# juicedata/juicefs

Measured on AMD Instinct MI355X. Metric: device-resident GiB/s (de)compress, 4 MiB blocks, LZ4+Zstd, 1/2/4/8 MI355X, higher is better.
Workload: dtype u8; 1 GPU; LZ4 decompress, 4096x4MiB blocks already in HBM (BASELINE configs[1]); blocks_per_gpu=4096, block_bytes=4194304, class=T, compressed_bytes_per_gpu=8570049795, parallelism=1 process(es), one per GPU, blocks sharded, no collective

## Files before the change

### juicefs_amd/csrc/lz4_decode.hip

```cpp
#include <hip/hip_runtime.h>
#include <stdint.h>

#include "jfs_internal.h"
#include "lz4_put16.h"
#include "lz4_tailpack.h"
#include "lz4_walkstep.h"
#include "wave.cuh"

namespace jfs {
namespace lz4d {

constexpr int P = 32;
constexpr int CW = 64 * P;
constexpr int CWIN = CW + 80;
constexpr int R = 4096;
constexpr int RMASK = R - 1;
constexpr int SEG = 128;
constexpr int TMAX = CW / 3 + 2;
constexpr int TCAP = 448 < TMAX ? 448 : TMAX;
#ifndef JFS_DIAG
#define JFS_DIAG 0
#endif
enum : unsigned {
    D_SKIP_ZERO = 1,
    D_SKIP_LIT = 2,
    D_SKIP_FAR = 4,
    D_SKIP_SUBST = 8,
    D_SKIP_NEAR = 16,
    D_PARSEONLY = 32,
    D_NOCOPY = 64,
};
constexpr unsigned DIAG = JFS_DIAG;
constexpr uint32_t STOP = 0x80000000u;
constexpr uint32_t NONE = 0xFFFFFFFFu;
constexpr int KEXT = 64;
constexpr int FLUSH_T = 1024;
constexpr int LMAX = 64;
constexpr int BSPAN = 2048;
static_assert(BSPAN + FLUSH_T + 128 <= R, "ring must hold the unflushed tail plus one batch");
static_assert(R - BSPAN >= LMAX + 16, "far sources must lie below the flushed prefix");
static_assert(R == (int)TP_RING && LMAX <= (int)TP_LEN_MAX, "tail_pack field widths (lz4_tailpack.h)");

#ifdef JFS_PROF
#define NPROF 30
__device__ uint64_t g_prof[NPROF];
struct Prof {
    uint64_t t, last, acc[NPROF];
    __device__ void start() {
        t = __builtin_amdgcn_s_memtime();
        for (int i = 0; i < NPROF; i++) acc[i] = 0;
    }
    __device__ void stamp(int k) {
        uint64_t x = __builtin_amdgcn_s_memtime();
        last = x - t;
        acc[k] += last;
        t = x;
    }
    __device__ void flush_out() {
        if (__lane_id() == 0)
            for (int i = 0; i < NPROF; i++) atomicAdd((unsigned long long *)&g_prof[i], acc[i]);
    }
};
#define PSTAMP(k) pr.stamp(k)
#define PCOUNT(k, n) (pr.acc[k] += (n))
#define PFIRST(...) __VA_ARGS__
#define PWALK(kind)                                                        \
    do {                                                                   \
        const uint64_t re_ = __ballot((kind) == WS_REDONE);                \
        pr.acc[26] += (uint64_t)__popcll(re_);                             \
        pr.acc[27] += re_ != 0;                                            \
        pr.acc[28] += (uint64_t)__popcll(__ballot((kind) == WS_ARRIVED)); \
    } while (0)
#define PROF_ARG , Prof &pr
#define PROF_PASS , pr
#else
#define PSTAMP(k)
#define PCOUNT(k, n)
#define PFIRST(...)
#define PWALK(kind) (void)(kind)
#define PROF_ARG
#define PROF_PASS
#endif

enum { W_NONE = 0, W_WIN = 1, W_SER = 2, W_BUG = 3 };
constexpr int32_t W_PFIRST = 16;
struct Meta {
    int32_t kind, wbase, cbase;
    uint32_t T, efin;
};
struct Ctl {
    int32_t done, restart, rip;
    int32_t step;
};

struct Smem {
    alignas(16) uint8_t ring[R];
    alignas(16) uint8_t cwin[2][CWIN];
    alignas(16) uint16_t tab[2][TCAP];
    Meta meta[2];
    Ctl ctl;
};

struct Ctx {
    const gc_u8 *src;
    g_u8 *dst;
    int32_t n;
    int32_t cap;
    int32_t F;
    int32_t Fw;
    uint32_t dmis;
    int32_t cbase;
    int32_t bug;
    uint8_t *cw;
    uint32_t cwoff;
    uint16_t *tab;
};

typedef uint32_t u32x4 __attribute__((ext_vector_type(4), aligned(4)));
typedef uint32_t u32x2 __attribute__((ext_vector_type(2), aligned(4)));
typedef JFS_GLOBAL const u32x4 gc_x4;
typedef JFS_GLOBAL const u32x2 gc_x2;

__device__ __forceinline__ uint32_t slot(const Ctx &c, int32_t pos) { return (uint32_t)(pos + (int32_t)c.dmis) & RMASK; }

template <bool UNDER>
__device__ __forceinline__ void far_load(const Ctx &c, uintptr_t a, uint32_t &d0, uint32_t &d1, uint32_t &d2,
                                         uint32_t &d3, uint32_t &d4, uint32_t &d5) {
    const uintptr_t b = a & ~(uintptr_t)3, lo = (uintptr_t)c.dst & ~(uintptr_t)3;
    const bool under = UNDER && b < lo;
    const gc_x4 *q = (const gc_x4 *)(under ? lo : b);
    const u32x4 v = q[0];
    const u32x2 w = *(const gc_x2 *)(q + 1);
    d0 = v.x; d1 = v.y; d2 = v.z; d3 = v.w; d4 = w.x; d5 = w.y;
    if (under) { d5 = d4; d4 = d3; d3 = d2; d2 = d1; d1 = d0; d0 = 0; }
}

__device__ __forceinline__ uint32_t cb(const Smem &s, const Ctx &c, int32_t p) {
    int32_t r = p - c.cbase;
    if ((uint32_t)r < (uint32_t)CWIN) return c.cw[r];
    return (p >= 0 && p < c.n) ? c.src[p] : 0u;
}

__device__ __forceinline__ void stage_window(Smem &s, Ctx &c, int32_t wbase) {
    const int l = lane_id();
    const uint32_t mis = (uint32_t)(((uintptr_t)c.src + (uint32_t)wbase) & 15u);
    c.cbase = wbase - (int32_t)mis;
    constexpr int NCH = (CWIN / 16 + 63) / 64;
    uint4 v[NCH];
#pragma unroll
    for (int j = 0; j < NCH; ++j) {
        const int k = l + 64 * j;
        const int32_t p = c.cbase + 16 * k;
        v[j] = make_uint4(0, 0, 0, 0);
        if (k < CWIN / 16 && p < c.n) v[j] = *(const gc_u4 *)(c.src + p);
    }
#pragma unroll
    for (int j = 0; j < NCH; ++j) {
        const int k = l + 64 * j;
        if (k < CWIN / 16) *(uint4 *)(c.cw + 16 * k) = v[j];
    }
    if (c.cbase < 0 || c.cbase + CWIN > c.n) {
        for (int k = l; k < CWIN; k += 64) {
            int32_t p = c.cbase + k;
            if (p >= c.n || p < 0) c.cw[k] = 0;
        }
    }
}

struct Tok {
    int32_t nxt;
    int32_t ll;
    int32_t ml;
    int32_t off;
    int32_t lit;
    int32_t llx;
};

__device__ __forceinline__ Tok parse_tok(const Smem &s, const Ctx &c, int32_t p) {
    Tok t;
    const int32_t n = c.n;
    t.ll = t.ml = t.off = t.lit = t.llx = 0;
    if (p > n - 18) { t.nxt = (int32_t)(STOP | (uint32_t)p); return t; }
    uint32_t tb = cb(s, c, p);
    int32_t q = p + 1;
    int32_t ll = (int32_t)(tb >> 4);
    if (ll == 15) {
        t.llx = 1;
        int k = 0;
        uint32_t sv;
        do {
            sv = cb(s, c, q);
            q++;
            ll += (int32_t)sv;
            if (q >= n - 15 || ++k > KEXT) { t.nxt = (int32_t)(STOP | (uint32_t)p); return t; }
        } while (sv == 255);
        if (q + ll > n - 32) { t.nxt = (int32_t)(STOP | (uint32_t)p); return t; }
    }
    t.lit = q;
    t.ll = ll;
    q += ll;
    t.off = (int32_t)(cb(s, c, q) | (cb(s, c, q + 1) << 8));
    q += 2;
    int32_t ml = (int32_t)(tb & 15);
    if (ml == 15) {
        int k = 0;
        uint32_t sv;
        do {
            sv = cb(s, c, q);
            q++;
            ml += (int32_t)sv;
            if (q >= n - 4 || ++k > KEXT) { t.nxt = (int32_t)(STOP | (uint32_t)p); return t; }
        } while (sv == 255);
    }
    t.ml = ml + 4;
    t.nxt = q;
    return t;
}

struct FTok {
    int32_t nxt, lit;
    uint32_t ll, ml, off, llx;
    bool slow, stop;
};

__device__ __forceinline__ uint32_t w8(const Ctx &c, int32_t r) { return c.cw[r < CWIN - 1 ? r : CWIN - 1]; }

__device__ __forceinline__ FTok parse_fast(const Smem &s, const Ctx &c, int32_t p) {
    FTok t;
    const int32_t n = c.n, b0 = c.cbase;
    const int32_t r = p - b0;
    const uint32_t tb = w8(c, r), e1 = w8(c, r + 1);
    const bool llx = (tb >> 4) == 15;
    int32_t q = r + 1 + (llx ? 1 : 0);
    t.ll = (tb >> 4) + (llx ? e1 : 0u);
    bool slow = llx && e1 == 255;
    bool stop = p > n - 18;
    stop |= llx && (b0 + q >= n - 15 || b0 + q + (int32_t)t.ll > n - 32);
    t.lit = b0 + q;
    q += (int32_t)t.ll;
    slow |= q + 3 > CWIN;
    const uint32_t o0 = w8(c, q), o1 = w8(c, q + 1), e2 = w8(c, q + 2);
    q += 2;
    const bool mlx = (tb & 15) == 15;
    t.ml = (tb & 15) + (mlx ? e2 : 0u) + 4;
    q += mlx ? 1 : 0;
    slow |= mlx && e2 == 255;
    stop |= mlx && b0 + q >= n - 4;
    t.off = o0 | (o1 << 8);
    t.llx = llx ? 1u : 0u;
    t.nxt = b0 + q;
    t.slow = slow;
    t.stop = stop;
    return t;
}

__device__ __forceinline__ void flush(Smem &s, Ctx &c, int32_t to) {
    const int l = lane_id();
    int32_t F = c.F;
    if (to <= F) return;
    int32_t a = F + (int32_t)((16u - ((c.dmis + (uint32_t)F) & 15u)) & 15u);
    if (a > to) a = to;
    if (l < a - F) c.dst[F + l] = s.ring[slot(c, F + l)];
    int32_t b = a + ((to - a) & ~15);
    for (int32_t x = a + 16 * l; x < b; x += 1024) {
        uint4 v = *(const uint4 *)(s.ring + slot(c, x));
        *(g_u4 *)(c.dst + x) = v;
    }
    if (l < to - b) c.dst[b + l] = s.ring[slot(c, b + l)];
    c.F = to;
}

__device__ __forceinline__ void flush_to_line(Smem &s, Ctx &c, int32_t hi) {
    int32_t to = (int32_t)(((uint32_t)hi + c.dmis) & ~127u) - (int32_t)c.dmis;
    if (to > c.F) flush(s, c, to);
}

__device__ __forceinline__ uint32_t out_byte(const Smem &s, const Ctx &c, int32_t x, int32_t ringfloor) {
    if (x >= ringfloor) return s.ring[slot(c, x)];
    return c.dst[x];
}

__device__ __forceinline__ void need_flushed(Ctx &c, int32_t lim) {
    if (lim > c.Fw) {
        wait_vm();
        c.Fw = c.F;
    }
}

constexpr int32_t LIT_DIRECT = 2 * R;
__device__ __forceinline__ void direct_lit(Smem &s, Ctx &c, int32_t srcpos, int32_t op, int32_t body) {
    const int l = lane_id();
    flush(s, c, op);
    const gc_u8 *sp = c.src + srcpos - op;
    int32_t x = op;
    const int32_t ha = (int32_t)((16u - (((uint32_t)(uintptr_t)(c.dst + x)) & 15u)) & 15u);
    if (l < ha) c.dst[x + l] = sp[x + l];
    x += ha;
    for (; x + 4096 <= body; x += 4096) {
        u32x4 v[4];
        uint32_t w[4];
        const uint32_t sh = (uint32_t)((uintptr_t)(sp + x) & 3u);
#pragma unroll
        for (int j = 0; j < 4; ++j) {
            const uintptr_t a = (uintptr_t)(sp + x + 1024 * j + 16 * l) & ~(uintptr_t)3;
            v[j] = *(const gc_x4 *)a;
            w[j] = *(const gc_u32 *)(a + 16);
        }
#pragma unroll
        for (int j = 0; j < 4; ++j) {
            uint4 o;
            o.x = __builtin_amdgcn_alignbyte(v[j].y, v[j].x, sh);
            o.y = __builtin_amdgcn_alignbyte(v[j].z, v[j].y, sh);
            o.z = __builtin_amdgcn_alignbyte(v[j].w, v[j].z, sh);
            o.w = __builtin_amdgcn_alignbyte(w[j], v[j].w, sh);
            *(g_u4 *)(c.dst + x + 1024 * j + 16 * l) = o;
        }
    }
    for (; x < body; x += 64)
        if (x + l < body) c.dst[x + l] = sp[x + l];
    c.F = body;
// ... 186 lines not shown
        if (rvl(c, &ip, n - 4, 1, 0, &length) != 0) goto err;
    }
    length += 4;
safe_match:
    st.fast = 0;
    if (match < 0) goto err;
    cpy = op + length;
    if (cpy > cap - 12 && cpy > cap - 5) goto err;
    coop_match(s, c, op, offset, (int32_t)length);
    op = (int32_t)cpy;
    st.ip = ip;
    st.op = op;
    return SER_CONT;
err:
    st.ip = ip;
    st.ret = -ip - 1;
    return SER_ERR;
}

__device__ __forceinline__ uint32_t lomask(int32_t k) {
    k = k < 0 ? 0 : k;
    return k >= 4 ? 0xFFFFFFFFu : ((1u << (8 * k)) - 1u);
}

__device__ __forceinline__ void lds_or(uint8_t *ring, uint32_t a, uint32_t v) {
    __hip_atomic_fetch_or(reinterpret_cast<uint32_t *>(ring) + (a >> 2), v, __ATOMIC_RELAXED,
                          __HIP_MEMORY_SCOPE_WORKGROUP);
}
__device__ __forceinline__ void lds_or_at(uint32_t *p, uint32_t v) {
    __hip_atomic_fetch_or(p, v, __ATOMIC_RELAXED, __HIP_MEMORY_SCOPE_WORKGROUP);
}

template <bool WRAP>
__device__ __forceinline__ void put16(Smem &s, uint32_t da, int32_t m, uint32_t w0, uint32_t w1, uint32_t w2,
                                      uint32_t w3, uint32_t w4) {
    uint8_t *ring = s.ring;
    const Put16Masks k = put16_masks(da & 3u, (uint32_t)m);
    if constexpr (WRAP) {
        const uint32_t D0 = da & ~3u;
        lds_or(ring, D0, w0 & k.k[0]);
        lds_or(ring, (D0 + 4) & RMASK, w1 & k.k[1]);
        lds_or(ring, (D0 + 8) & RMASK, w2 & k.k[2]);
        lds_or(ring, (D0 + 12) & RMASK, w3 & k.k[3]);
        lds_or(ring, (D0 + 16) & RMASK, w4 & k.k[4]);
    } else {
        uint32_t *p = reinterpret_cast<uint32_t *>(ring) + (da >> 2);
        lds_or_at(p, w0 & k.k[0]);
        lds_or_at(p + 1, w1 & k.k[1]);
        lds_or_at(p + 2, w2 & k.k[2]);
        lds_or_at(p + 3, w3 & k.k[3]);
        lds_or_at(p + 4, w4 & k.k[4]);
    }
}

template <bool WRAP>
__device__ __forceinline__ void zero_span(Smem &s, const Ctx &c, int32_t O0, int32_t O1) {
    const int l = lane_id();
    const uint32_t a = slot(c, O0), h = a & 3u;
    if (l == 0 && h)
        __hip_atomic_fetch_and(reinterpret_cast<uint32_t *>(s.ring) + (a >> 2), lomask((int32_t)h), __ATOMIC_RELAXED,
                               __HIP_MEMORY_SCOPE_WORKGROUP);
    if constexpr (WRAP) {
        const int32_t A = O0 + (int32_t)((4u - h) & 3u);
        for (int32_t x = A + 4 * l; x < O1; x += 256) *(uint32_t *)(s.ring + slot(c, x)) = 0u;
    } else {
        const uint32_t e = a + (uint32_t)(O1 - O0);
        for (uint32_t x = ((a + 3u) & ~3u) + 4u * (uint32_t)l; x < e; x += 256) *(uint32_t *)(s.ring + x) = 0u;
    }
}

template <bool RING, bool WRAP>
__device__ __forceinline__ void copy16(Smem &s, uint32_t sa, uint32_t da, int32_t m) {
    const uint8_t *lds = (const uint8_t *)&s;
    const uint32_t ha = da & 3u;
    const uint32_t sb = RING ? (sa - ha) & RMASK : sa - ha, S0 = sb & ~3u, sh = sb & 3u;
    uint32_t r[6];
    if (RING && __ballot(S0 > (uint32_t)(R - 24))) {
#pragma unroll
        for (int j = 0; j < 6; ++j) r[j] = *(const uint32_t *)(lds + ((S0 + 4 * j) & RMASK));
    } else {
#pragma unroll
        for (int j = 0; j < 6; ++j) r[j] = *(const uint32_t *)(lds + S0 + 4 * j);
    }
    put16<WRAP>(s, da, m, __builtin_amdgcn_alignbyte(r[1], r[0], sh), __builtin_amdgcn_alignbyte(r[2], r[1], sh),
                __builtin_amdgcn_alignbyte(r[3], r[2], sh), __builtin_amdgcn_alignbyte(r[4], r[3], sh),
                __builtin_amdgcn_alignbyte(r[5], r[4], sh));
}


template <bool WRAP>
__device__ __forceinline__ void wave_near(Smem &s, uint32_t ds, uint32_t ss, int32_t len) {
    const int l = lane_id();
    const int32_t D = (int32_t)((ds - ss) & RMASK);
    const int32_t step = D < 64 ? D : 64;
    if (!WRAP && ss + (uint32_t)len <= (uint32_t)R) {
        const int32_t back = (int32_t)ss - (int32_t)ds;
        uint8_t *d = s.ring + ds + l;
        for (int32_t left = len; left > 0; left -= step, d += step)
            if (l < (left < step ? left : step)) d[0] = d[back];
        return;
    }
    for (int32_t k = 0; k < len; k += step) {
        const int32_t i = k + l;
        if (l < step && i < len) s.ring[(ds + (uint32_t)i) & RMASK] = s.ring[(ds + (uint32_t)(i - D)) & RMASK];
    }
}
__device__ __forceinline__ void wave_lit(Smem &s, const Ctx &c, int32_t op, uint32_t litr, int32_t from, int32_t len) {
    const int l = lane_id();
    for (int32_t k = from; k < len; k += 64) {
        const int32_t i = k + l;
        if (i < len) s.ring[slot(c, op + i)] = c.cw[litr + (uint32_t)i];
    }
}

template <bool WRAP>
__device__ __forceinline__ void batch(Smem &s, Ctx &c, bool act, int32_t o, uint32_t ll, uint32_t ml, uint32_t off,
                                      uint32_t litr, int32_t O0, int32_t O1 PROF_ARG) {
    const int32_t hz = O1 + 4 - R;
    asm volatile("" : "+v"(o));
    PCOUNT(14, 1);
    if (O0 - c.F >= FLUSH_T) flush_to_line(s, c, O0);
    if constexpr (!(DIAG & D_SKIP_ZERO)) zero_span<WRAP>(s, c, O0, O1);
    const int32_t ms = o + (int32_t)ll, msrc = ms - (int32_t)off;
    const uint32_t sbias = c.dmis - (((uint32_t)O0 + c.dmis) & ~(uint32_t)RMASK);
    auto dslot = [&](int32_t pos) -> uint32_t { return WRAP ? slot(c, pos) : (uint32_t)pos + sbias; };
    const bool hasm = act && ml > 0;
    const bool zero = hasm && off == 0;
    const bool far = hasm && off != 0 && msrc < hz;
    if (__ballot(far) && hz + LMAX > c.Fw) {
        wait_vm();
        c.Fw = c.F;
        if (hz + LMAX > c.Fw) c.bug = 4;
    }
    uint32_t fd0 = 0, fd1 = 0, fd2 = 0, fd3 = 0, fd4 = 0, fd5 = 0;
    const uint32_t fha = slot(c, ms) & 3u;
    if (__ballot(far)) {
        if (__ballot(far && msrc < 4)) {
            if (far) far_load<true>(c, (uintptr_t)(c.dst + msrc) - fha, fd0, fd1, fd2, fd3, fd4, fd5);
        } else {
            if (far) far_load<false>(c, (uintptr_t)(c.dst + msrc) - fha, fd0, fd1, fd2, fd3, fd4, fd5);
        }
    }
    for (uint32_t k = 0; !(DIAG & D_SKIP_LIT) && __ballot(act && k < ll); k += 16) {
        PCOUNT(16, 1);
        if (act && k < ll) {
            const int32_t m = ll - k < 16u ? (int32_t)(ll - k) : 16;
            copy16<false, WRAP>(s, c.cwoff + litr + k, dslot(o + (int32_t)k), m);
        }
    }
    PSTAMP(4);
    if (!(DIAG & D_SKIP_FAR) && __ballot(far)) {
        for (uint32_t k = 0; __ballot(far && k < ml); k += 16) {
            PCOUNT(17, 1);
            if (far && k < ml) {
                const int32_t m = ml - k < 16u ? (int32_t)(ml - k) : 16;
                const uint32_t da = dslot(ms + (int32_t)k);
                const uint32_t sh = (uint32_t)((uintptr_t)(c.dst + msrc + (int32_t)k) - fha) & 3u;
                put16<WRAP>(s, da, m, __builtin_amdgcn_alignbyte(fd1, fd0, sh),
                            __builtin_amdgcn_alignbyte(fd2, fd1, sh), __builtin_amdgcn_alignbyte(fd3, fd2, sh),
                            __builtin_amdgcn_alignbyte(fd4, fd3, sh), __builtin_amdgcn_alignbyte(fd5, fd4, sh));
            }
            const bool more = far && k + 16 < ml;
            if (__ballot(more)) {
                if (more)
                    far_load<false>(c, (uintptr_t)(c.dst + msrc + (int32_t)k + 16) - fha, fd0, fd1, fd2, fd3, fd4, fd5);
            }
        }
    }
    PSTAMP(5);
    bool pend = hasm && !far && !zero;
    int32_t src = msrc;
    const uint64_t am = __ballot(act);
    const int first = am ? (int)__builtin_ctzll(am) : 0;
    const uint32_t key = act ? (uint32_t)ms : (lane_id() < first ? 0u : 0xFFFFFFFFu);
    bool litsrc = false;
    {
        const uint32_t mek = pend ? (uint32_t)(ms + (int32_t)ml) : 0u;
        const bool want = !(DIAG & D_SKIP_SUBST) && pend && off >= ml && src >= O0;
        if (__ballot(want)) {
            int lo = 0;
#pragma unroll
            for (int stp = 32; stp; stp >>= 1) {
                const uint32_t v = (uint32_t)__shfl((int)key, lo + stp, 64);
                lo = v <= (uint32_t)src ? lo + stp : lo;
            }
            const uint32_t vms = (uint32_t)__shfl((int)key, lo, 64);
            const uint32_t vme = (uint32_t)__shfl((int)mek, lo, 64);
            const int32_t voff = __shfl((int)off, lo, 64);
            const bool ok = want && vms <= (uint32_t)src && (uint32_t)(src + (int32_t)ml) <= vme && voff > 0 &&
                            src - voff >= hz;
            const uint32_t nms = (uint32_t)__shfl((int)key, lo + 1 < 64 ? lo + 1 : 63, 64);
            litsrc = want && vms <= (uint32_t)src && (uint32_t)src >= vme && lo < 63 &&
                     (uint32_t)(src + (int32_t)ml) <= nms;
            src = ok ? src - voff : src;
        }
    }
    int32_t pos = ms, rem = (int32_t)ml, D = ms - src;
    const int32_t send = src + (int32_t)ml < ms ? src + (int32_t)ml : ms;
    if (!(DIAG & D_SKIP_NEAR)) {
        PCOUNT(18, 1);
        const bool go = pend && (send <= O0 || litsrc);
        if (__ballot(go)) {
            PCOUNT(15, 1);
            if (go) {
                const int32_t m = rem < 16 ? (rem < D ? rem : D) : (D < 16 ? D : 16);
                copy16<true, WRAP>(s, slot(c, pos - D), dslot(pos), m);
                pos += m;
                rem -= m;
                if (rem <= 0) pend = false;
            }
        }
        const uint32_t tw = tail_pack(dslot(pos), slot(c, pos - D), (uint32_t)rem, (uint32_t)D);
        for (uint64_t pmk = __ballot(pend); pmk;) {
            const int j = (int)__builtin_ctzll(pmk);
            pmk &= ~(1ull << j);
            PCOUNT(19, 1);
            const uint32_t w = readlane(tw, j);
            if (tail_direct(w)) {
                if ((uint32_t)lane_id() < tail_rem(w)) s.ring[tail_ds(w) + lane_id()] = s.ring[tail_ss(w) + lane_id()];
            } else {
                wave_near<WRAP>(s, tail_ds(w), tail_ss(w), (int32_t)tail_rem(w));
            }
        }
    }
    PSTAMP(6);
}

__device__ __forceinline__ uint32_t copy_tokens(Smem &s, Ctx &c, uint32_t T, int32_t op0, int32_t *end_op,
                                                int32_t *bad_ip PROF_ARG) {
    const int l = lane_id();
    int32_t op = op0;
    const int32_t cap = c.cap;
    if constexpr ((DIAG & D_PARSEONLY) != 0) {
        *end_op = op0;
        return T;
    }
    for (uint32_t g0 = 0; g0 < T; g0 += 64) {
        const uint32_t n0 = T - g0 < 64u ? T - g0 : 64u;
        const bool in0 = (uint32_t)l < n0;
        const int32_t p = c.cbase + (in0 ? (int32_t)c.tab[g0 + l] : 0);
        FTok t = parse_fast(s, c, p);
        const bool sl = in0 && t.slow;
        if (__ballot(sl)) {
            if (sl) {
                const Tok u = parse_tok(s, c, p);
                t.lit = u.lit;
                t.ll = (uint32_t)u.ll;
                t.ml = (uint32_t)u.ml;
                t.off = (uint32_t)u.off;
                t.llx = (uint32_t)u.llx;
            }
        }
        const uint32_t ll = in0 ? t.ll : 0u, ml = in0 ? t.ml : 0u, off = t.off;
        const uint32_t litr = (uint32_t)(t.lit - c.cbase);
        const uint32_t len = ll + ml;
        const uint32_t incl = dpp_scan_add(len);
        const int32_t o = op + (int32_t)(incl - len);
        const int32_t om = o + (int32_t)ll;
        const bool bad = in0 && ((t.llx && om > cap - 32) || (om + (int32_t)ml >= cap - 64) || ((int32_t)off > om));
        const uint64_t bm = __ballot(bad);
        const uint32_t n = bm ? (uint32_t)__builtin_ctzll(bm) : n0;
        const bool in = (uint32_t)l < n;
        const int32_t endo = o + (int32_t)len;
        const bool lng = in && (ll > (uint32_t)LMAX || ml > (uint32_t)LMAX);
        PSTAMP(2);
        uint32_t j = 0;
        while (j < n) {
            const int32_t oj = (int32_t)readlane((uint32_t)o, (int)j);
            if (readlane(lng ? 1u : 0u, (int)j)) {
                const uint32_t jll = readlane(ll, (int)j), jml = readlane(ml, (int)j), joff = readlane(off, (int)j);
                const uint32_t jlit = readlane(litr, (int)j);
                coop_lit(s, c, c.cbase + (int32_t)jlit, oj, (int32_t)jll);
                coop_match(s, c, oj + (int32_t)jll, (int32_t)joff, (int32_t)jml);
                PSTAMP(7);
                j++;
                continue;
            }
            const bool ok = (uint32_t)l >= j && in && !lng && endo - oj <= BSPAN;
            const uint64_t stop = __ballot(!ok) & (~0ull << j);
            const uint32_t e = stop ? (uint32_t)__builtin_ctzll(stop) : 64u;
            const uint32_t eb = e > n ? n : e;
            const bool act = (uint32_t)l >= j && (uint32_t)l < eb;
            const int32_t O1 = (int32_t)readlane((uint32_t)endo, (int)eb - 1);
            PSTAMP(3);
            if constexpr (!(DIAG & D_NOCOPY)) {
                if (slot(c, oj) + (uint32_t)(O1 - oj) + 20u <= (uint32_t)R)
                    batch<false>(s, c, act, o, ll, ml, off, litr, oj, O1 PROF_PASS);
                else
                    batch<true>(s, c, act, o, ll, ml, off, litr, oj, O1 PROF_PASS);
            }
            j = eb;
        }
        if (bm) {
            *bad_ip = (int32_t)readlane((uint32_t)p, (int)n);
            *end_op = (int32_t)readlane((uint32_t)o, (int)n);
            return g0 + n;
        }
        op += (int32_t)readlane(incl, 63);
    }
    *end_op = op;
    return T;
}

static_assert(SEG == 128, "segment bit sets are two u64 per lane");
constexpr int SW = 64 * SEG;
constexpr int SPRE = 32;
constexpr int SEG_BUDGET = 64;
constexpr int SEG_MIN = 4;

static_assert(WS_STOP == STOP && WS_KEXT == KEXT, "lz4_walkstep.h restates the parser's constants");
__device__ __noinline__ uint32_t g_next_exact(const Ctx &c, int32_t p) {
    return ws_next_exact([&](uint32_t i) { return (uint32_t)c.src[i]; }, c.n, p);
}


struct SegWalk {
    int32_t base, plo, phi;
    int32_t q;
    uint32_t cur;
    uint32_t sx, ex;
    uint64_t vs0, vs1;
    uint64_t vt0, vt1;
    uint64_t vp0, vp1;
    bool mv;
    uint32_t pe2;
    bool pend;
    int phase;
    bool round;
    int steps, rounds;

    __device__ __forceinline__ void start(int32_t b) {
        const int l = lane_id();
        base = b;
        plo = b + l * SEG;
        phi = plo + SEG;
        cur = l == 0 ? (uint32_t)b : (uint32_t)(plo - SPRE);
        q = (int32_t)cur;
        vs0 = vs1 = vt0 = vt1 = vp0 = vp1 = 0;
        sx = ex = 0;
        mv = true;
        pe2 = 0;
        pend = false;
        phase = 0;
        round = false;
        steps = rounds = 0;
    }

    __device__ __forceinline__ bool advance(Ctx &c, int budget PROF_ARG) {
        const auto fetch = [&](uint32_t i) { return (uint32_t)c.src[i]; };
        const auto exact = [&](int32_t p) { return g_next_exact(c, p); };
        if (phase == 0) {
            for (; budget > 0 && __ballot(mv); --budget) {
                PCOUNT(11, 1);
                int kind = WS_STEPPED;
                if (mv) kind = ws_spec_iter(*this, fetch, exact, c.n);
                PWALK(kind);
                if (++steps > SEG + SPRE) { c.bug = 6; phase = 2; return true; }
            }
            if (budget == 0) return false;
            vt0 = vs0;
            vt1 = vs1;
            ex = sx;
            phase = 1;
            round = true;
        }
        while (phase == 1 && budget > 0) {
            if (round) {
                const uint32_t In = dpp_shift_up(ex, (uint32_t)base);
                const bool ch = In != cur;
                if (!__ballot(ch)) { phase = 2; break; }
                if (++rounds > 64) { c.bug = 3; phase = 2; break; }
                PCOUNT(12, 1);
                mv = false;
                if (ch) {
                    cur = In;
                    const uint32_t d = In - (uint32_t)plo;
                    if ((In & STOP) || (int32_t)In >= phi) {
                        vt0 = vt1 = 0;
                        ex = In;
                    } else if (tbit2(vs0, vs1, d)) {
                        vt0 = vs0 & from_lo(d);
                        vt1 = vs1 & from_hi(d);
                        ex = sx;
                    } else {
                        mv = true;
                    }
                }
                q = (int32_t)In;
                vp0 = vp1 = 0;
                steps = 0;
                round = false;
            }
            for (; budget > 0 && __ballot(mv); --budget) {
                PCOUNT(13, 1);
                int kind = WS_STEPPED;
                if (mv) kind = ws_fix_iter(*this, fetch, exact, c.n);
                PWALK(kind);
                if (++steps > SEG + 1) { c.bug = 7; phase = 2; return true; }
            }
            if (!__ballot(mv)) round = true;
        }
        return phase == 2;
    }
};

__device__ __forceinline__ uint32_t span_dword(uint64_t vt0, uint64_t vt1, int32_t k) {
    const int src = (k >> 2) & 63;
    const uint32_t d0 = (uint32_t)__shfl((int)(uint32_t)vt0, src, 64);
    const uint32_t d1 = (uint32_t)__shfl((int)(uint32_t)(vt0 >> 32), src, 64);
    const uint32_t d2 = (uint32_t)__shfl((int)(uint32_t)vt1, src, 64);
    const uint32_t d3 = (uint32_t)__shfl((int)(uint32_t)(vt1 >> 32), src, 64);
    const uint32_t j = (uint32_t)k & 3u;
    const uint32_t v = j == 0 ? d0 : j == 1 ? d1 : j == 2 ? d2 : d3;
    return (k >= 0 && k < 4 * 64) ? v : 0u;
}

struct Span {
    uint64_t v0, v1;
    int32_t base;
    uint32_t exit;
};

__device__ __forceinline__ void parse_window_seg(Smem &s, Ctx &c, int32_t wbase, const Span &sp, uint32_t *T_out,
                                                 uint32_t *efin_out PROF_ARG) {
    static_assert(P == 32, "a window lane covers one dword of the span bit set");
    const int l = lane_id();
    stage_window(s, c, wbase);
    const int32_t cbase = c.cbase;
    PCOUNT(10, 1);
    __builtin_amdgcn_wave_barrier();
    PSTAMP(0);
    const int32_t send = sp.base + SW;
    const int32_t wend = cbase + CW < send ? cbase + CW : send;
    const int32_t o = cbase - sp.base + 32 * l;
    const int32_t K = o >> 5;
    const uint32_t lo = span_dword(sp.v0, sp.v1, K), hi = span_dword(sp.v0, sp.v1, K + 1);
    uint32_t field = __builtin_amdgcn_alignbit(hi, lo, (uint32_t)o & 31u);
    const int32_t plo = cbase + 32 * l;
    const int32_t a = wbase - plo, b = wend - plo;
    const uint32_t ma = a <= 0 ? 0xFFFFFFFFu : a >= 32 ? 0u : (0xFFFFFFFFu << a);
    const uint32_t mb = b >= 32 ? 0xFFFFFFFFu : b <= 0 ? 0u : ((1u << b) - 1u);
    field &= ma & mb;
    PSTAMP(1);
    const uint32_t cnt = (uint32_t)__builtin_popcount(field);
    const uint32_t cinc = dpp_scan_add(cnt);
    const uint32_t tall = readlane(cinc, 63);
    *T_out = tall < (uint32_t)TCAP ? tall : (uint32_t)TCAP;
    uint32_t ex = 0;
    {
        uint32_t idx = cinc - cnt;
        uint32_t v = field;
        while (__ballot(v != 0)) {
            if (v) {
                const uint32_t bb = (uint32_t)__builtin_ctz(v);
                if (idx < (uint32_t)TCAP) c.tab[idx] = (uint16_t)((uint32_t)l * P + bb);
                else if (idx == (uint32_t)TCAP) ex = (uint32_t)plo + bb;
                idx++;
                v &= v - 1;
            }
        }
    }
    if (tall > (uint32_t)TCAP) {
        const uint64_t hit = __ballot(cinc - cnt <= (uint32_t)TCAP && (uint32_t)TCAP < cinc);
        *efin_out = readlane(ex, (int)__builtin_ctzll(hit));
    } else if (wend >= send) {
        *efin_out = sp.exit;
    } else {
        const int32_t d = wend - sp.base - l * SEG;
        const uint32_t dd = d < 0 ? 0u : (uint32_t)d;
        const uint64_t m0 = d >= SEG ? 0ull : sp.v0 & from_lo(dd), m1 = d >= SEG ? 0ull : sp.v1 & from_hi(dd);
        const uint64_t any = __ballot((m0 | m1) != 0ull);
        if (any) {
            const int f = (int)__builtin_ctzll(any);
            const uint32_t bit = m0 ? (uint32_t)__builtin_ctzll(m0) : 64u + (uint32_t)__builtin_ctzll(m1 | (1ull << 63));
            *efin_out = (uint32_t)sp.base + (uint32_t)(f * SEG) + readlane(bit, f);
        } else {
            *efin_out = sp.exit;
        }
    }
    PSTAMP(2);
}

__device__ __forceinline__ void wg_sync() { asm volatile("s_waitcnt lgkmcnt(0)\n\ts_barrier" ::: "memory"); }

__device__ __forceinline__ void use_buffer(Smem &s, Ctx &c, int buf) {
    c.cw = s.cwin[buf];
    c.cwoff = (uint32_t)((const uint8_t *)s.cwin[buf] - (const uint8_t *)&s);
    c.tab = s.tab[buf];
}

__device__ __forceinline__ void parser_wave(Smem &s, Ctx &c PROF_ARG) {
    int32_t pip = 0;
    bool pstop = false;
    Span sp;
    sp.v0 = sp.v1 = 0;
    sp.base = 0;
    sp.exit = 0;
    bool spv = false;
    bool nxt = false;
    SegWalk wk;
    wk.start(0);
    for (uint32_t k = 0;; ++k) {
        const int buf = (int)(k & 1u);
        Meta m;
        m.kind = W_NONE;
        m.wbase = pip;
        m.cbase = 0;
        m.T = 0;
        m.efin = 0;
        PFIRST(bool pfirst = false);
        if (!pstop) {
            if (pip < c.n - 64) {
                use_buffer(s, c, buf);
                uint32_t T, efin;
                if (!spv || pip >= sp.base + SW) {
                    if (!(spv && nxt && wk.base == pip)) wk.start(pip);
                    PFIRST(const uint64_t it0 = pr.acc[11] + pr.acc[13]; pfirst = true);
                    wk.advance(c, 1 << 20 PROF_PASS);
                    PSTAMP(1);
                    PFIRST(const uint64_t its = pr.acc[11] + pr.acc[13] - it0; pr.acc[22] += 1; pr.acc[23] += its;
                           pr.acc[24] += pr.last; pr.acc[25] += its == 0);
                    sp.v0 = wk.vt0;
                    sp.v1 = wk.vt1;
                    sp.base = pip;
                    sp.exit = readlane(wk.ex, 63);
                    spv = true;
                    nxt = !(sp.exit & STOP) && !c.bug;
                    if (nxt) wk.start((int32_t)sp.exit);
                }
                parse_window_seg(s, c, pip, sp, &T, &efin PROF_PASS);
                if (nxt) {
                    bool fin = wk.advance(c, SEG_MIN PROF_PASS);
                    for (int g = SEG_MIN; !fin && g < SEG_BUDGET; g += 2) {
                        if (__hip_atomic_load(&s.ctl.step, __ATOMIC_RELAXED, __HIP_MEMORY_SCOPE_WORKGROUP) >= (int32_t)k)
                            break;
                        fin = wk.advance(c, 2 PROF_PASS);
                    }
                }
                PSTAMP(1);
                m.kind = c.bug ? W_BUG : W_WIN;
                PFIRST(if (pfirst && !c.bug) m.kind |= W_PFIRST);
                m.cbase = c.cbase;
                m.T = T;
                m.efin = efin;
                if ((efin & STOP) || c.bug) pstop = true;
                else pip = (int32_t)efin;
            } else {
                m.kind = W_SER;
                pstop = true;
            }
        }
        if (lane_id() == 0) s.meta[buf] = m;
        wg_sync();
        const int32_t done = (int32_t)uniform((uint32_t)s.ctl.done), restart = (int32_t)uniform((uint32_t)s.ctl.restart),
                      rip = (int32_t)uniform((uint32_t)s.ctl.rip);
        wg_sync();
        PSTAMP(9);
        PFIRST(if (pfirst) pr.acc[21] += pr.last);
        if (done) break;
        if (restart) {
            pip = rip;
            pstop = false;
            spv = false;
            nxt = false;
        }
    }
}

template <bool PREFIX>
__device__ __forceinline__ void copier_wave(Smem &s, Ctx &c, int32_t *retp, int32_t want PROF_ARG) {
    __builtin_amdgcn_s_setprio(1);
    Ser st;
    st.ip = 0;
    st.op = 0;
    st.fast = c.cap >= 64;
    st.ret = 0;
    bool skip = false;
    int32_t result = INT32_MIN;
    int64_t nser = 0;
    PFIRST(uint64_t wait8 = 0);
    if (lane_id() == 0) __hip_atomic_store(&s.ctl.step, -1, __ATOMIC_RELAXED, __HIP_MEMORY_SCOPE_WORKGROUP);
    for (uint32_t k = 0;; ++k) {
        int32_t done = 0, restart = 0, rip = 0;
        if (k > 0 && !skip) {
            const int buf = (int)((k - 1) & 1u);
            Meta m;
            m.kind = (int32_t)uniform((uint32_t)s.meta[buf].kind);
            PFIRST(if (m.kind & W_PFIRST) pr.acc[20] += wait8; m.kind &= ~W_PFIRST);
            m.wbase = (int32_t)uniform((uint32_t)s.meta[buf].wbase);
            m.cbase = (int32_t)uniform((uint32_t)s.meta[buf].cbase);
            m.T = uniform(s.meta[buf].T);
            m.efin = uniform(s.meta[buf].efin);
            bool ser = false;
            if (m.kind == W_BUG || m.kind == W_NONE || m.wbase != st.ip) {
                c.bug |= 8;
            } else if (m.kind == W_WIN && st.fast && st.ip < c.n - 64 && st.op < c.cap - 128) {
                use_buffer(s, c, buf);
                c.cbase = m.cbase;
                int32_t end_op = st.op, bad_ip = 0;
                const uint32_t dn = m.T > 0 ? copy_tokens(s, c, m.T, st.op, &end_op, &bad_ip PROF_PASS) : 0u;
                st.op = end_op;
                if (dn < m.T) {
                    st.ip = bad_ip;
                    ser = true;
                } else {
                    st.ip = (int32_t)(m.efin & ~STOP);
                    ser = (m.efin & STOP) != 0;
                }
                if constexpr (PREFIX) {
                    if (st.op >= want) {
                        ser = false;
                        flush(s, c, st.op);
                        result = want;
                        done = 1;
                    }
                }
            } else {
                ser = true;
            }
            if (ser && !c.bug) {
                c.cbase = 0x3fffffff;
                for (;;) {
                    const int status = ser_seq(s, c, st);
                    if (status != SER_CONT) {
                        if (status == SER_DONE) flush(s, c, st.op);
                        result = st.ret;
                        if constexpr (PREFIX) result = st.ret > want ? want : st.ret;
                        done = 1;
                        break;
                    }
                    if constexpr (PREFIX) {
                        if (st.op >= want) {
                            flush(s, c, st.op);
                            result = want;
                            done = 1;
                            break;
                        }
                    }
                    if (++nser > (int64_t)c.n + 64) { c.bug |= 16; break; }
                    if (st.fast && st.ip < c.n - 64 && st.op < c.cap - 128) {
                        restart = 1;
                        rip = st.ip;
                        break;
                    }
                }
                PSTAMP(7);
            }
            if (c.bug) {
                done = 1;
                restart = 0;
                result = INT32_MIN;
            }
        }
        if (k > (uint32_t)c.n + 64) {
            done = 1;
            result = INT32_MIN;
        }
        if (lane_id() == 0) {
            s.ctl.done = done;
            s.ctl.restart = restart;
            s.ctl.rip = rip;
            __hip_atomic_store(&s.ctl.step, (int32_t)k, __ATOMIC_RELAXED, __HIP_MEMORY_SCOPE_WORKGROUP);
        }
        wg_sync();
        wg_sync();
        PSTAMP(8);
        PFIRST(wait8 = pr.last);
        if (done) break;
        skip = restart != 0;
    }
    if (lane_id() == 0) *retp = result;
}

#define JFS_LZ4_ATTR __attribute__((amdgpu_num_sgpr(80), amdgpu_waves_per_eu(8)))
template <bool PREFIX, class... WANT>
__global__ __launch_bounds__(128) JFS_LZ4_ATTR void lz4_decode_kernel(const jfs_dev_block *__restrict__ blocks, int nblk,
                                                        int32_t *__restrict__ ret,
                                                        const int32_t *__restrict__ lens,
                                                        const int32_t *__restrict__ todo, WANT... wantp) {
    static_assert(sizeof...(WANT) == (PREFIX ? 1 : 0), "the prefix instantiation takes want, the full one does not");
    __shared__ Smem s;
    const int b = blockIdx.x;
    if (b >= nblk) return;
    if (todo && !todo[b]) return;
    const int wave = (int)uniform(threadIdx.x >> 6);
    jfs_dev_block d = ((const gc_blk *)blocks)[b];
    Ctx c;
    c.src = (const gc_u8 *)d.src;
    c.dst = (g_u8 *)d.dst;
    c.n = lens ? lens[b] : d.src_len;
    if (lens && c.n < 0) {
        if (threadIdx.x == 64) ret[b] = JFS_CHAIN_FAILED;
        return;
    }
    c.cap = d.dst_cap;
    c.F = 0;
    c.Fw = 0;
    c.dmis = (uint32_t)((uintptr_t)d.dst & 15u);
    c.cbase = 0x3fffffff;
    c.bug = 0;
    use_buffer(s, c, 0);
#ifdef JFS_PROF
    Prof pr;
    pr.start();
#endif
    int32_t early = 1, result = 0;
    if (d.src == nullptr || c.n < 0 || c.cap < 0) result = -1;
    else if (c.cap == 0) result = (c.n == 1 && c.src[0] == 0) ? 0 : -1;
    else if (c.n == 0) result = -1;
    else early = 0;
    if (early) {
        if (wave == 1 && lane_id() == 0) ret[b] = result;
        return;
    }
    int32_t want = 0;
    if constexpr (PREFIX) {
        want = (int32_t)uniform((uint32_t)(wantp, ...)[b]);
        if (want <= 0) {
            if (wave == 1 && lane_id() == 0) ret[b] = 0;
            return;
        }
        if (want > c.cap) want = c.cap;
    }
    if (wave == 0) parser_wave(s, c PROF_PASS);
    else copier_wave<PREFIX>(s, c, ret + b, want PROF_PASS);
#ifdef JFS_PROF
    pr.flush_out();
#endif
}

}
}

#ifndef JFS_LZ4_DECODE_PREFIX_TU
#ifdef JFS_PROF
extern "C" int jfs_prof_read(uint64_t *out) {
    return hipMemcpyFromSymbol(out, HIP_SYMBOL(jfs::lz4d::g_prof), sizeof(uint64_t) * NPROF) == hipSuccess ? 0 : -1;
}
extern "C" int jfs_prof_reset() {
    uint64_t z[NPROF] = {0};
    return hipMemcpyToSymbol(HIP_SYMBOL(jfs::lz4d::g_prof), z, sizeof(z)) == hipSuccess ? 0 : -1;
}
#endif

extern "C" int jfs_launch_lz4_decode(const jfs_dev_block *d_blocks, int nblk, int32_t *d_ret, hipStream_t stream) {
    return jfs_launch_lz4_decode_lens(d_blocks, nblk, d_ret, nullptr, stream);
}

extern "C" int jfs_launch_lz4_decode_lens(const jfs_dev_block *d_blocks, int nblk, int32_t *d_ret, const int32_t *d_lens,
                                          hipStream_t stream) {
    if (nblk <= 0) return 0;
    hipLaunchKernelGGL(jfs::lz4d::lz4_decode_kernel<false>, dim3(nblk), dim3(128), 0, stream, d_blocks, nblk, d_ret,
                       d_lens, (const int32_t *)nullptr);
    return hipGetLastError() == hipSuccess ? 0 : -1;
}

extern "C" int jfs_launch_lz4_decode_todo(const jfs_dev_block *d_blocks, int nblk, int32_t *d_ret, const int32_t *d_todo,
                                          hipStream_t stream) {
    if (nblk <= 0) return 0;
    hipLaunchKernelGGL(jfs::lz4d::lz4_decode_kernel<false>, dim3(nblk), dim3(128), 0, stream, d_blocks, nblk, d_ret,
                       (const int32_t *)nullptr, d_todo);
    return hipGetLastError() == hipSuccess ? 0 : -1;
}

#else
extern "C" int jfs_launch_lz4_decode_prefix(const jfs_dev_block *d_blocks, int nblk, int32_t *d_ret,
                                            const int32_t *d_want, const int32_t *d_todo, hipStream_t stream) {
    if (nblk <= 0) return 0;
    hipLaunchKernelGGL((jfs::lz4d::lz4_decode_kernel<true, const int32_t *>), dim3(nblk), dim3(128), 0, stream,
                       d_blocks, nblk, d_ret, (const int32_t *)nullptr, d_todo, d_want);
    return hipGetLastError() == hipSuccess ? 0 : -1;
}
#endif
```

### juicefs_amd/csrc/lz4_walkstep.h

```cpp
#pragma once
#include <stdint.h>

#if defined(__HIPCC__)
#define JFS_WALKSTEP_HD __host__ __device__ __forceinline__
#else
#define JFS_WALKSTEP_HD inline
#endif

namespace jfs {
namespace lz4d {

constexpr uint32_t WS_STOP = 0x80000000u;
constexpr int WS_KEXT = 64;

template <class F>
JFS_WALKSTEP_HD uint32_t ws_next_exact(F fetch, int32_t n, int32_t p) {
    if (p > n - 18) return WS_STOP | (uint32_t)p;
    const uint32_t tb = fetch((uint32_t)p);
    int32_t q = p + 1;
    int32_t ll = (int32_t)(tb >> 4);
    if (ll == 15) {
        int k = 0;
        uint32_t sv;
        do {
            sv = fetch((uint32_t)q);
            q++;
            ll += (int32_t)sv;
            if (q >= n - 15 || ++k > WS_KEXT) return WS_STOP | (uint32_t)p;
        } while (sv == 255);
        if (q + ll > n - 32) return WS_STOP | (uint32_t)p;
    }
    q += ll + 2;
    if ((tb & 15u) == 15u) {
        int k = 0;
        uint32_t sv;
        do {
            sv = fetch((uint32_t)q);
            q++;
            if (q >= n - 4 || ++k > WS_KEXT) return WS_STOP | (uint32_t)p;
        } while (sv == 255);
    }
    return (uint32_t)q;
}

struct WsRound {
    uint32_t x;
    uint32_t q;
    uint32_t halt;
    uint32_t ext;
    uint32_t mlx;
};
template <class F>
JFS_WALKSTEP_HD WsRound ws_round(F fetch, int32_t n, int32_t p, uint32_t &pe2) {
    const uint32_t edge = (uint32_t)(p > n - 18);
    const uint32_t up = (uint32_t)p;
    uint32_t tb = fetch(edge ? 0u : up), e1 = fetch(edge ? 0u : up + 1u);
#if defined(__HIP_DEVICE_COMPILE__)
    asm volatile("" : "+v"(tb), "+v"(e1), "+v"(pe2));
#endif
    const uint32_t hi = tb >> 4;
    const uint32_t llx = (uint32_t)(hi == 15u);
    const uint32_t L = llx ? 15u + e1 : hi;
    const uint32_t lstop = llx & ((uint32_t)(p + 2 >= n - 15) | (uint32_t)(p + 2 + (int32_t)L > n - 32));
    WsRound r;
    r.q = up + 3u + llx + L;
    r.mlx = (uint32_t)((tb & 15u) == 15u);
    r.x = r.q + r.mlx;
    r.halt = edge | lstop;
    r.ext = (r.halt ^ 1u) & llx & (uint32_t)(e1 == 255u);
    return r;
}

JFS_WALKSTEP_HD bool tbit2(uint64_t a0, uint64_t a1, uint32_t d) {
    return (((d < 64u ? a0 : a1) >> (d & 63u)) & 1ull) != 0;
}
JFS_WALKSTEP_HD void sbit2(uint64_t &a0, uint64_t &a1, uint32_t d) {
    const uint64_t m = 1ull << (d & 63u);
    a0 |= d < 64u ? m : 0ull;
    a1 |= d < 64u ? 0ull : m;
}
JFS_WALKSTEP_HD void pbit2(uint64_t &a0, uint64_t &a1, uint32_t d, bool on) {
    const uint64_t m = 1ull << (d & 63u);
    uint64_t &a = d < 64u ? a0 : a1;
    a = on ? a | m : a & ~m;
}
JFS_WALKSTEP_HD uint64_t from_lo(uint32_t d) { return d < 64u ? (~0ull << (d & 63u)) : 0ull; }
JFS_WALKSTEP_HD uint64_t from_hi(uint32_t d) { return d < 64u ? ~0ull : (~0ull << (d & 63u)); }

enum { WS_STEPPED = 0, WS_REDONE = 1, WS_ARRIVED = 2 };

template <class W, class F>
JFS_WALKSTEP_HD uint32_t ws_take(W &w, uint32_t &pp, const WsRound &r, F fetch, int32_t n, bool *ext) {
    const uint32_t last = r.mlx & (uint32_t)((int32_t)r.x >= n - 4);
    const uint32_t pend = (r.halt ^ 1u) & (r.ext ^ 1u) & r.mlx & (last ^ 1u);
    w.pe2 = fetch(pend ? r.q : 0u);
    pp = (uint32_t)w.q;
    w.pend = pend != 0;
    *ext = r.ext != 0;
    return (r.halt | last) ? (WS_STOP | (uint32_t)w.q) : r.x;
}

template <class W, class F, class X>
JFS_WALKSTEP_HD int ws_spec_iter(W &w, F fetch, X exact, int32_t n) {
    const WsRound r = ws_round(fetch, n, w.q, w.pe2);
    const bool redo = w.pend && w.pe2 == 255u;
    const bool arr = w.pend && !redo && w.q >= w.phi;
    const int32_t at = redo ? (int32_t)w.sx : w.q;
    uint32_t x = (uint32_t)w.q;
    bool ex = redo;
    if (redo || arr) w.pend = false;
    else x = ws_take(w, w.sx, r, fetch, n, &ex);
    if (ex) x = exact(at);
    const bool stop = (x & WS_STOP) != 0;
    if (!arr && at >= w.plo) pbit2(w.vs0, w.vs1, (uint32_t)(at - w.plo), !stop);
    const bool out = stop || (!w.pend && (int32_t)x >= w.phi);
    w.sx = out ? x : w.sx;
    w.mv = !out;
    w.q = (int32_t)x;
    return redo ? WS_REDONE : arr ? WS_ARRIVED : WS_STEPPED;
}

template <class W, class F, class X>
JFS_WALKSTEP_HD int ws_fix_iter(W &w, F fetch, X exact, int32_t n) {
    const WsRound r = ws_round(fetch, n, w.q, w.pe2);
    const bool redo = w.pend && w.pe2 == 255u;
    const bool arr = w.pend && !redo && w.q >= w.phi;
    const int32_t at = redo ? (int32_t)w.ex : w.q;
    const uint32_t d = (uint32_t)(at - w.plo);
    const bool join = !redo && !arr && tbit2(w.vs0, w.vs1, d);
    uint32_t x = (uint32_t)w.q;
    bool ex = redo;
    if (redo || arr || join) w.pend = false;
    else x = ws_take(w, w.ex, r, fetch, n, &ex);
    if (ex) x = exact(at);
    const bool stop = (x & WS_STOP) != 0;
    if (!arr && !join) pbit2(w.vp0, w.vp1, d, !stop);
    const bool out = join || stop || (!w.pend && (int32_t)x >= w.phi);
    if (out) {
        w.vt0 = w.vp0 | (join ? w.vs0 & from_lo(d) : 0ull);
        w.vt1 = w.vp1 | (join ? w.vs1 & from_hi(d) : 0ull);
        w.ex = join ? w.sx : x;
    }
    w.mv = !out;
    w.q = (int32_t)x;
    return redo ? WS_REDONE : arr ? WS_ARRIVED : WS_STEPPED;
}

}
}
```

Baseline: 509.2 GiB/s.

## Double LZ4 parse-walk segment width to 256 bytes per lane using generic bitsets

Each lane's speculative token-boundary walk now covers a 256-byte segment instead of 128, and the segment bit sets become a templated BitSet holding four u64 words. One wave's span then covers 16 KiB, so fewer span walks and join rounds are needed per block. The fix-up pass also drops the separate vp bit set and builds the result directly in vt. In exchange, each lane walks a longer serial chain, spends more registers on the bit sets, and does more shuffles per span dword, which can lower occupancy or add walk latency.

After: 534.8 GiB/s, median of 6. +5.0%, better.

```diff
diff --git a/juicefs_amd/csrc/lz4_decode.hip b/juicefs_amd/csrc/lz4_decode.hip
--- a/juicefs_amd/csrc/lz4_decode.hip
+++ b/juicefs_amd/csrc/lz4_decode.hip
@@ -15,7 +15,10 @@
 constexpr int CWIN = CW + 80;
 constexpr int R = 4096;
 constexpr int RMASK = R - 1;
-constexpr int SEG = 128;
+#ifndef JFS_LZ4_WALK_SEG
+#define JFS_LZ4_WALK_SEG 256
+#endif
+constexpr int SEG = JFS_LZ4_WALK_SEG;
 constexpr int TMAX = CW / 3 + 2;
 constexpr int TCAP = 448 < TMAX ? 448 : TMAX;
 #ifndef JFS_DIAG
@@ -808,7 +811,8 @@
     return T;
 }
 
-static_assert(SEG == 128, "segment bit sets are two u64 per lane");
+static_assert(SEG == 128 || SEG == 256, "a lane's segment bit set: two or four u64 (BitSet, lz4_walkstep.h)");
+using SegBits = BitSet<SEG>;
 constexpr int SW = 64 * SEG;
 constexpr int SPRE = 32;
 constexpr int SEG_BUDGET = 64;
@@ -825,9 +829,8 @@
     int32_t q;
     uint32_t cur;
     uint32_t sx, ex;
-    uint64_t vs0, vs1;
-    uint64_t vt0, vt1;
-    uint64_t vp0, vp1;
+    SegBits vs;
+    SegBits vt;
     bool mv;
     uint32_t pe2;
     bool pend;
@@ -842,7 +845,8 @@
         phi = plo + SEG;
         cur = l == 0 ? (uint32_t)b : (uint32_t)(plo - SPRE);
         q = (int32_t)cur;
-        vs0 = vs1 = vt0 = vt1 = vp0 = vp1 = 0;
+        vs.clear();
+        vt.clear();
         sx = ex = 0;
         mv = true;
         pe2 = 0;
@@ -859,13 +863,12 @@
             for (; budget > 0 && __ballot(mv); --budget) {
                 PCOUNT(11, 1);
                 int kind = WS_STEPPED;
-                if (mv) kind = ws_spec_iter(*this, fetch, exact, c.n);
+                if (mv) kind = ws_spec_iter(*this, vs, fetch, exact, c.n);
                 PWALK(kind);
                 if (++steps > SEG + SPRE) { c.bug = 6; phase = 2; return true; }
             }
             if (budget == 0) return false;
-            vt0 = vs0;
-            vt1 = vs1;
+            vt = vs;
             ex = sx;
             phase = 1;
             round = true;
@@ -882,25 +885,24 @@
                     cur = In;
                     const uint32_t d = In - (uint32_t)plo;
                     if ((In & STOP) || (int32_t)In >= phi) {
-                        vt0 = vt1 = 0;
+                        vt.clear();
                         ex = In;
-                    } else if (tbit2(vs0, vs1, d)) {
-                        vt0 = vs0 & from_lo(d);
-                        vt1 = vs1 & from_hi(d);
+                    } else if (vs.test(d)) {
+                        vt = vs.and_from(d);
                         ex = sx;
                     } else {
+                        vt.clear();
                         mv = true;
                     }
                 }
                 q = (int32_t)In;
-                vp0 = vp1 = 0;
                 steps = 0;
                 round = false;
             }
             for (; budget > 0 && __ballot(mv); --budget) {
                 PCOUNT(13, 1);
                 int kind = WS_STEPPED;
-                if (mv) kind = ws_fix_iter(*this, fetch, exact, c.n);
+                if (mv) kind = ws_fix_iter(*this, vs, vt, fetch, exact, c.n);
                 PWALK(kind);
                 if (++steps > SEG + 1) { c.bug = 7; phase = 2; return true; }
             }
@@ -910,19 +912,21 @@
     }
 };
 
-__device__ __forceinline__ uint32_t span_dword(uint64_t vt0, uint64_t vt1, int32_t k) {
-    const int src = (k >> 2) & 63;
-    const uint32_t d0 = (uint32_t)__shfl((int)(uint32_t)vt0, src, 64);
-    const uint32_t d1 = (uint32_t)__shfl((int)(uint32_t)(vt0 >> 32), src, 64);
-    const uint32_t d2 = (uint32_t)__shfl((int)(uint32_t)vt1, src, 64);
-    const uint32_t d3 = (uint32_t)__shfl((int)(uint32_t)(vt1 >> 32), src, 64);
-    const uint32_t j = (uint32_t)k & 3u;
-    const uint32_t v = j == 0 ? d0 : j == 1 ? d1 : j == 2 ? d2 : d3;
-    return (k >= 0 && k < 4 * 64) ? v : 0u;
+__device__ __forceinline__ uint32_t span_dword(const SegBits &v, int32_t k) {
+    constexpr int DW = SEG / 32;
+    const int src = (k >> (DW == 4 ? 2 : 3)) & 63;
+    const uint32_t j = (uint32_t)k & (uint32_t)(DW - 1);
+    uint32_t r = 0;
+    ws_each<DW>([&](auto i) {
+        const uint32_t di = (uint32_t)(v.w[i.v >> 1] >> (32 * (i.v & 1)));
+        const uint32_t got = (uint32_t)__shfl((int)di, src, 64);
+        r = j == (uint32_t)i.v ? got : r;
+    });
+    return (k >= 0 && k < DW * 64) ? r : 0u;
 }
 
 struct Span {
-    uint64_t v0, v1;
+    SegBits v;
     int32_t base;
     uint32_t exit;
 };
@@ -940,7 +944,7 @@
     const int32_t wend = cbase + CW < send ? cbase + CW : send;
     const int32_t o = cbase - sp.base + 32 * l;
     const int32_t K = o >> 5;
-    const uint32_t lo = span_dword(sp.v0, sp.v1, K), hi = span_dword(sp.v0, sp.v1, K + 1);
+    const uint32_t lo = span_dword(sp.v, K), hi = span_dword(sp.v, K + 1);
     uint32_t field = __builtin_amdgcn_alignbit(hi, lo, (uint32_t)o & 31u);
     const int32_t plo = cbase + 32 * l;
     const int32_t a = wbase - plo, b = wend - plo;
@@ -973,12 +977,10 @@
         *efin_out = sp.exit;
     } else {
         const int32_t d = wend - sp.base - l * SEG;
-        const uint32_t dd = d < 0 ? 0u : (uint32_t)d;
-        const uint64_t m0 = d >= SEG ? 0ull : sp.v0 & from_lo(dd), m1 = d >= SEG ? 0ull : sp.v1 & from_hi(dd);
-        const uint64_t any = __ballot((m0 | m1) != 0ull);
+        const uint32_t bit = sp.v.first_from(d < 0 ? 0u : (uint32_t)d);
+        const uint64_t any = __ballot(bit < (uint32_t)SEG);
         if (any) {
             const int f = (int)__builtin_ctzll(any);
-            const uint32_t bit = m0 ? (uint32_t)__builtin_ctzll(m0) : 64u + (uint32_t)__builtin_ctzll(m1 | (1ull << 63));
             *efin_out = (uint32_t)sp.base + (uint32_t)(f * SEG) + readlane(bit, f);
         } else {
             *efin_out = sp.exit;
@@ -999,7 +1001,7 @@
     int32_t pip = 0;
     bool pstop = false;
     Span sp;
-    sp.v0 = sp.v1 = 0;
+    sp.v.clear();
     sp.base = 0;
     sp.exit = 0;
     bool spv = false;
@@ -1026,8 +1028,7 @@
                     PSTAMP(1);
                     PFIRST(const uint64_t its = pr.acc[11] + pr.acc[13] - it0; pr.acc[22] += 1; pr.acc[23] += its;
                            pr.acc[24] += pr.last; pr.acc[25] += its == 0);
-                    sp.v0 = wk.vt0;
-                    sp.v1 = wk.vt1;
+                    sp.v = wk.vt;
                     sp.base = pip;
                     sp.exit = readlane(wk.ex, 63);
                     spv = true;
diff --git a/juicefs_amd/csrc/lz4_walkstep.h b/juicefs_amd/csrc/lz4_walkstep.h
--- a/juicefs_amd/csrc/lz4_walkstep.h
+++ b/juicefs_amd/csrc/lz4_walkstep.h
@@ -71,21 +71,68 @@
     return r;
 }
 
-JFS_WALKSTEP_HD bool tbit2(uint64_t a0, uint64_t a1, uint32_t d) {
-    return (((d < 64u ? a0 : a1) >> (d & 63u)) & 1ull) != 0;
-}
-JFS_WALKSTEP_HD void sbit2(uint64_t &a0, uint64_t &a1, uint32_t d) {
-    const uint64_t m = 1ull << (d & 63u);
-    a0 |= d < 64u ? m : 0ull;
-    a1 |= d < 64u ? 0ull : m;
-}
-JFS_WALKSTEP_HD void pbit2(uint64_t &a0, uint64_t &a1, uint32_t d, bool on) {
-    const uint64_t m = 1ull << (d & 63u);
-    uint64_t &a = d < 64u ? a0 : a1;
-    a = on ? a | m : a & ~m;
-}
-JFS_WALKSTEP_HD uint64_t from_lo(uint32_t d) { return d < 64u ? (~0ull << (d & 63u)) : 0ull; }
-JFS_WALKSTEP_HD uint64_t from_hi(uint32_t d) { return d < 64u ? ~0ull : (~0ull << (d & 63u)); }
+template <int I>
+struct WsIdx {
+    static constexpr int v = I;
+};
+template <int K, int I = 0, class Fn>
+JFS_WALKSTEP_HD void ws_each(Fn f) {
+    if constexpr (I < K) {
+        f(WsIdx<I>());
+        ws_each<K, I + 1>(f);
+    }
+}
+
+template <int N>
+struct BitSet {
+    static_assert(N > 0 && N % 64 == 0, "whole u64 words");
+    static constexpr int W = N / 64;
+    uint64_t w[W];
+
+    JFS_WALKSTEP_HD void clear() {
+        ws_each<W>([&](auto i) { w[i.v] = 0ull; });
+    }
+    JFS_WALKSTEP_HD bool test(uint32_t d) const {
+        uint64_t a = w[0];
+        ws_each<W>([&](auto i) { a = i.v > 0 && d >= 64u * (uint32_t)i.v ? w[i.v] : a; });
+        return ((a >> (d & 63u)) & 1ull) != 0;
+    }
+    JFS_WALKSTEP_HD void put(uint32_t d, bool on) {
+        const uint64_t m = 1ull << (d & 63u);
+        ws_each<W>([&](auto i) {
+            const uint64_t v = on ? w[i.v] | m : w[i.v] & ~m;
+            w[i.v] = (d >> 6) == (uint32_t)i.v ? v : w[i.v];
+        });
+    }
+    static JFS_WALKSTEP_HD BitSet from(uint32_t d) {
+        BitSet r;
+        const uint64_t part = ~0ull << (d & 63u);
+        ws_each<W>([&](auto i) { r.w[i.v] = (d >> 6) < (uint32_t)i.v ? ~0ull : (d >> 6) == (uint32_t)i.v ? part : 0ull; });
+        return r;
+    }
+    JFS_WALKSTEP_HD BitSet and_from(uint32_t d) const {
+        BitSet r = from(d);
+        ws_each<W>([&](auto i) { r.w[i.v] &= w[i.v]; });
+        return r;
+    }
+    JFS_WALKSTEP_HD void or_in(const BitSet &o) {
+        ws_each<W>([&](auto i) { w[i.v] |= o.w[i.v]; });
+    }
+    JFS_WALKSTEP_HD bool any() const {
+        uint64_t a = 0ull;
+        ws_each<W>([&](auto i) { a |= w[i.v]; });
+        return a != 0ull;
+    }
+    JFS_WALKSTEP_HD uint32_t first_from(uint32_t d) const {
+        const BitSet m = and_from(d);
+        uint32_t r = (uint32_t)N;
+        ws_each<W>([&](auto i) {
+            constexpr int k = W - 1 - i.v;
+            r = m.w[k] ? 64u * (uint32_t)k + (uint32_t)__builtin_ctzll(m.w[k] | (1ull << 63)) : r;
+        });
+        return r;
+    }
+};
 
 enum { WS_STEPPED = 0, WS_REDONE = 1, WS_ARRIVED = 2 };
 
@@ -100,8 +147,8 @@
     return (r.halt | last) ? (WS_STOP | (uint32_t)w.q) : r.x;
 }
 
-template <class W, class F, class X>
-JFS_WALKSTEP_HD int ws_spec_iter(W &w, F fetch, X exact, int32_t n) {
+template <int N, class W, class F, class X>
+JFS_WALKSTEP_HD int ws_spec_iter(W &w, BitSet<N> &vs, F fetch, X exact, int32_t n) {
     const WsRound r = ws_round(fetch, n, w.q, w.pe2);
     const bool redo = w.pend && w.pe2 == 255u;
     const bool arr = w.pend && !redo && w.q >= w.phi;
@@ -112,7 +159,7 @@
     else x = ws_take(w, w.sx, r, fetch, n, &ex);
     if (ex) x = exact(at);
     const bool stop = (x & WS_STOP) != 0;
-    if (!arr && at >= w.plo) pbit2(w.vs0, w.vs1, (uint32_t)(at - w.plo), !stop);
+    if (!arr && at >= w.plo) vs.put((uint32_t)(at - w.plo), !stop);
     const bool out = stop || (!w.pend && (int32_t)x >= w.phi);
     w.sx = out ? x : w.sx;
     w.mv = !out;
@@ -120,31 +167,60 @@
     return redo ? WS_REDONE : arr ? WS_ARRIVED : WS_STEPPED;
 }
 
-template <class W, class F, class X>
-JFS_WALKSTEP_HD int ws_fix_iter(W &w, F fetch, X exact, int32_t n) {
+template <int N, class W, class F, class X>
+JFS_WALKSTEP_HD int ws_fix_iter(W &w, const BitSet<N> &vs, BitSet<N> &vt, F fetch, X exact, int32_t n) {
     const WsRound r = ws_round(fetch, n, w.q, w.pe2);
     const bool redo = w.pend && w.pe2 == 255u;
     const bool arr = w.pend && !redo && w.q >= w.phi;
     const int32_t at = redo ? (int32_t)w.ex : w.q;
     const uint32_t d = (uint32_t)(at - w.plo);
-    const bool join = !redo && !arr && tbit2(w.vs0, w.vs1, d);
+    const bool join = !redo && !arr && vs.test(d);
     uint32_t x = (uint32_t)w.q;
     bool ex = redo;
     if (redo || arr || join) w.pend = false;
     else x = ws_take(w, w.ex, r, fetch, n, &ex);
     if (ex) x = exact(at);
     const bool stop = (x & WS_STOP) != 0;
-    if (!arr && !join) pbit2(w.vp0, w.vp1, d, !stop);
+    if (!arr && !join) vt.put(d, !stop);
+    if (join) vt.or_in(vs.and_from(d));
     const bool out = join || stop || (!w.pend && (int32_t)x >= w.phi);
-    if (out) {
-        w.vt0 = w.vp0 | (join ? w.vs0 & from_lo(d) : 0ull);
-        w.vt1 = w.vp1 | (join ? w.vs1 & from_hi(d) : 0ull);
-        w.ex = join ? w.sx : x;
-    }
+    if (out) w.ex = join ? w.sx : x;
     w.mv = !out;
     w.q = (int32_t)x;
     return redo ? WS_REDONE : arr ? WS_ARRIVED : WS_STEPPED;
 }
 
-}
-}
+JFS_WALKSTEP_HD BitSet<128> ws_set2(uint64_t a0, uint64_t a1) {
+    BitSet<128> s;
+    s.w[0] = a0;
+    s.w[1] = a1;
+    return s;
+}
+JFS_WALKSTEP_HD bool tbit2(uint64_t a0, uint64_t a1, uint32_t d) { return ws_set2(a0, a1).test(d); }
+JFS_WALKSTEP_HD void sbit2(uint64_t &a0, uint64_t &a1, uint32_t d) {
+    BitSet<128> s = ws_set2(a0, a1);
+    s.put(d, true);
+    a0 = s.w[0];
+    a1 = s.w[1];
+}
+JFS_WALKSTEP_HD uint64_t from_lo(uint32_t d) { return BitSet<128>::from(d).w[0]; }
+JFS_WALKSTEP_HD uint64_t from_hi(uint32_t d) { return BitSet<128>::from(d).w[1]; }
+template <class W, class F, class X>
+JFS_WALKSTEP_HD int ws_spec_iter(W &w, F fetch, X exact, int32_t n) {
+    BitSet<128> vs = ws_set2(w.vs0, w.vs1);
+    const int kind = ws_spec_iter(w, vs, fetch, exact, n);
+    w.vs0 = vs.w[0];
+    w.vs1 = vs.w[1];
+    return kind;
+}
+template <class W, class F, class X>
+JFS_WALKSTEP_HD int ws_fix_iter(W &w, F fetch, X exact, int32_t n) {
+    BitSet<128> vt = ws_set2(w.vt0, w.vt1);
+    const int kind = ws_fix_iter(w, ws_set2(w.vs0, w.vs1), vt, fetch, exact, n);
+    w.vt0 = vt.w[0];
+    w.vt1 = vt.w[1];
+    return kind;
+}
+
+}
+}
```
